# aicell-lab/bioengine-worker

Hardware: AMD Instinct MI355X
Metric: cellpose_cyto3_512x512_imgs_per_sec (higher is better)
Workload: dtype bf16; 1 GPU; model=cellpose-cyto3 CPnet (nbase 2-32-64-128-256, style on, BN folded), global_batch=32, parallelism=dp1 (replica per GPU)

## Files before the change

bioengine_worker_amd/models/cpnet.py:

```python
from __future__ import annotations

import torch
import torch.nn as nn
import torch.nn.functional as F

import os

from ..ops import conv as convops
from ..ops import conv_pair as pairops
from ..ops import style as styleops


def _norm(c: int, kind: str) -> nn.Module:
    if kind == "batch":
        return nn.BatchNorm2d(c, eps=1e-5, momentum=0.05)
    if kind == "group":
        g = 8 if c % 8 == 0 else 1
        return nn.GroupNorm(g, c, eps=1e-5)
    raise ValueError(kind)


def batchconv(cin, cout, sz, norm="batch"):
    return nn.Sequential(_norm(cin, norm), nn.ReLU(inplace=True), nn.Conv2d(cin, cout, sz, padding=sz // 2))

# ... 115 lines not shown
        T0 = self.downsample(data)
        style = self.make_style(T0[-1])
        style0 = style
        if not self.style_on:
            style = style * 0
        T1 = self.upsample(style, T0)
        T1 = self.output(T1)
        return T1, style0, T0

    def randomize_(self, seed: int = 0) -> "CPnet":
        g = torch.Generator().manual_seed(seed)
        for m in self.modules():
            if isinstance(m, nn.Conv2d):
                fan_in = m.in_channels * m.kernel_size[0] * m.kernel_size[1]
                m.weight.data = torch.randn(m.weight.shape, generator=g) * (1.0 / fan_in) ** 0.5
                if m.bias is not None:
                    m.bias.data = torch.randn(m.bias.shape, generator=g) * 0.01
            elif isinstance(m, nn.Linear):
                m.weight.data = torch.randn(m.weight.shape, generator=g) * (1.0 / m.in_features) ** 0.5
                m.bias.data = torch.randn(m.bias.shape, generator=g) * 0.01
            elif isinstance(m, nn.BatchNorm2d):
                m.weight.data = 1.0 + 0.1 * torch.randn(m.weight.shape, generator=g)
                m.bias.data = 0.1 * torch.randn(m.bias.shape, generator=g)
                m.running_mean.data = 0.1 * torch.randn(m.running_mean.shape, generator=g)
                m.running_var.data = 1.0 + 0.1 * torch.rand(m.running_var.shape, generator=g)
            elif isinstance(m, nn.GroupNorm):
                m.weight.data = 1.0 + 0.1 * torch.randn(m.weight.shape, generator=g)
                m.bias.data = 0.1 * torch.randn(m.bias.shape, generator=g)
        return self



def _bn_fold(bn: nn.Module, device) -> tuple[torch.Tensor, torch.Tensor]:
    if isinstance(bn, nn.BatchNorm2d):
        s = bn.weight.detach().float() / torch.sqrt(bn.running_var.detach().float() + bn.eps)
        t = bn.bias.detach().float() - bn.running_mean.detach().float() * s
        return s.to(device).contiguous(), t.to(device).contiguous()
    raise TypeError("CPnetEngine folds eval-mode BatchNorm only; GroupNorm nets run the autograd path")


def _pad_vec(v: torch.Tensor, n: int, fill: float) -> torch.Tensor:
    if v.numel() == n:
        return v
    out = torch.full((n,), fill, dtype=v.dtype, device=v.device)
    out[: v.numel()] = v
    return out


class _FConv:

    def __init__(self, seq: nn.Sequential, relu: bool, device, cin_pad=None, cout_pad_to=None):
        bn, conv = seq[0], seq[-1]
        self.pc = convops.PackedConv.from_weight(conv.weight, conv.bias, cin_pad=cin_pad, cout_pad_to=cout_pad_to).to(device)
        if (convops.frag_eligible(self.pc) or convops.frag_eligible_pool(self.pc) or
                convops.frag_eligible_proj(self.pc)) and torch.device(device).type == "cuda":
            self.pc.frag()
        s, t = _bn_fold(bn, device)
        self.scale = _pad_vec(s, self.pc.cin_pad, 0.0)
        self.shift = _pad_vec(t, self.pc.cin_pad, 0.0)
        self.relu = relu

    def __call__(self, x, *, x2=None, shift=None, residual=None, inmode="none", out_nchw_f32=False, cout_valid=None,
                 residual_mode="full"):
        return convops.fused_conv2d(x, self.pc, x2=x2, scale=self.scale, shift=self.shift if shift is None else shift,
                                    relu=self.relu, residual=residual, inmode=inmode, out_nchw_f32=out_nchw_f32,
                                    cout_valid=cout_valid, residual_mode=residual_mode)


class _PPConv:

    def __init__(self, conv: nn.Conv2d, device):
        from ..ops import gemm_pp as ppops

        self.cout = conv.weight.shape[0]
        self.wp = ppops.pack_conv3(conv.weight).to(device)
        self.bias = None if conv.bias is None else conv.bias.detach().float().to(device).contiguous()
        cfg = os.environ.get("BE_CPNET_PP_CFG")
        self.cfg = None if cfg is None else int(cfg)


def _igc(x, pk, **kw):
    if isinstance(pk, _PPConv):
        from ..ops import gemm_pp as ppops

        return ppops.conv3(x, pk.wp, pk.bias, cfg=pk.cfg, **kw)
    from ..ops import conv_igemm as igops

    return igops.conv3_igemm(x, pk, **kw)


class CPnetEngine:

    def __init__(self, net: CPnet, device):
        net = net.eval()
        self.device = torch.device(device)
        self.nout = net.nout
        self.nchan = net.nchan
        self.cin_pad = convops._round_up(net.nchan, 8)
        d = self.device
        self.down = []
        for n, blk in enumerate(net.downsample.down):
            cin_pad = self.cin_pad if n == 0 else None
            self.down.append(dict(
                proj=_FConv(blk.proj, False, d, cin_pad),
                c0=_FConv(blk.conv[0], True, d, cin_pad),
                c1=_FConv(blk.conv[1], True, d),
                c2=_FConv(blk.conv[2], True, d),
                c3=_FConv(blk.conv[3], True, d),
# ... 80 lines not shown
                if cfg in pairops.PROJ_CONFIGS:
                    sp.frag_proj(sp.pa.wp.device)
        return pairs

    def _build_igemm(self, net: CPnet) -> dict:
        from ..ops import conv_igemm as igops
        from ..ops import gemm_pp as ppops

        ig = {}

        def add(key, conv: nn.Conv2d):
            cout, cin, kh, _ = conv.weight.shape
            if self.ig_kind == "pp":
                if kh == 3 and ppops.conv3_supported(cin, cout):
                    ig[key] = _PPConv(conv, self.device)
            elif kh == 3 and cin % 16 == 0 and cout % 64 == 0:
                ig[key] = igops.IgemmConv.from_weight(conv.weight, conv.bias).to(self.device)

        nup = len(net.upsample.up)
        for n, blk in enumerate(net.downsample.down):
            if ("down", n, 0) in self.pair or n == 0:
                continue
            for k in (1, 2, 3):
                add(("down", n, k), blk.conv[k][-1])
        for i, blk in enumerate(net.upsample.up):
            if ("up", i, 0) in self.pair:
                continue
            if i == nup - 1:
                add(("up", i, 0), blk.conv[0][-1])
            for k in (1, 2, 3):
                add(("up", i, k), blk.conv[k].conv[-1])
        levels = {}
        for (kind, idx, k) in ig:
            levels.setdefault((kind, idx), set()).add(k)
        full = {lv for lv, ks in levels.items() if ks >= {1, 2, 3}}
        only = os.environ.get("BE_CPNET_IGEMM_LEVELS", "3")
        if only:
            keep = {int(v) for v in only.split(",") if v.strip()}
            full = {lv for lv in full if lv[1] in keep}
        return {key: v for key, v in ig.items() if (key[0], key[1]) in full}

    def _ig_level(self, kind: str, idx: int, x: torch.Tensor, H: int, W: int) -> bool:
        from ..ops import conv_igemm as igops

        pk = self.ig.get((kind, idx, 1))
        if pk is None or not x.is_cuda:
            return False
        if isinstance(pk, _PPConv):
            return True
        return igops.supported(x.shape[0], H, W, pk.cout, pk.bn)

    def _down_ig(self, n: int, e: dict, src: torch.Tensor, next_act=None) -> torch.Tensor:
        ig = self.ig
        proj = e["proj"](src, inmode="pool2")
        c1, c2, c3 = e["c1"], e["c2"], e["c3"]
        ha = convops.fused_conv2d(src, e["c0"].pc, scale=e["c0"].scale, shift=e["c0"].shift, relu=True, inmode="pool2",
                                  post_scale=c1.scale, post_shift=c1.shift, post_relu=True)
        x1, x1a = _igc(ha, ig[("down", n, 1)], residual=proj, ascale=c2.scale, ashift=c2.shift)
        _, h2a = _igc(x1a, ig[("down", n, 2)], want_out=False, ascale=c3.scale, ashift=c3.shift)
        if next_act is None:
            xd, _ = _igc(h2a, ig[("down", n, 3)], residual=x1)
            return xd, None
        return _igc(h2a, ig[("down", n, 3)], residual=x1, ascale=next_act[0], ashift=next_act[1])

    def _up_ig(self, i: int, e: dict, xcur: torch.Tensor, y: torch.Tensor, shifts: dict, xcur_act=None):
        ig = self.ig
        c1, c2, c3 = e["c1"], e["c2"], e["c3"]
        if ("up", i, 0) in ig:
            proj = e["proj"](xcur)
            _, h0a = _igc(xcur_act, ig[("up", i, 0)], residual=y, want_out=False, ascale=c1.scale,
                                       ashift=shifts[(i, 1)])
        else:
            proj = e["proj"](xcur, inmode="up2")
            h0a = convops.fused_conv2d(xcur, e["c0"].pc, scale=e["c0"].scale, shift=e["c0"].shift, relu=True,
                                       inmode="up2", residual=y, post_scale=c1.scale, post_shift=shifts[(i, 1)],
                                       post_relu=True)
        x1, x1a = _igc(h0a, ig[("up", i, 1)], residual=proj, ascale=c2.scale, ashift=shifts[(i, 2)])
        _, h2a = _igc(x1a, ig[("up", i, 2)], want_out=False, ascale=c3.scale, ashift=shifts[(i, 3)])
        out, _ = _igc(h2a, ig[("up", i, 3)], residual=x1)
        return out

    def _style_shifts(self, style: torch.Tensor) -> dict:
        st = style if self.style_on else torch.zeros_like(style)
        return self._split_shifts(styleops.style_shifts(st, self.style_w, self.style_b, self.style_s, self.style_t))

    def _split_shifts(self, shifts_all: torch.Tensor) -> dict:
        out = {}
        for (i, k, off, c) in self._feat_slices:
            out[(i, k)] = shifts_all[:, off: off + c]
        return out

    @torch.no_grad()
    def forward(self, x: torch.Tensor):
        xd = []
        h = x
        P = self.pair
        nup = len(self.up)
        top_act = None
        for n, e in enumerate(self.down):
            im = "pool2" if n > 0 else "none"
            src = x if n == 0 else xd[-1]
            if n > 0 and ("down", n, 1) in self.ig and self._ig_level("down", n, src, src.shape[1] // 2,
                                                                       src.shape[2] // 2):
                last = n == len(self.down) - 1 and ("up", nup - 1, 0) in self.ig
                nxt = (self.up[nup - 1]["c0"].scale, self.up[nup - 1]["c0"].shift) if last else None
                xdn, top_act = self._down_ig(n, e, src, nxt)
                xd.append(xdn)
                continue
            if ("down", n, 0) in P:
                if n == 0:
# ... 59 lines not shown
```

bioengine_worker_amd/ops/conv.py:

```python
from __future__ import annotations

import os

from dataclasses import dataclass

import torch
import torch.nn.functional as F

from . import _native

CK_1X1 = 64

INMODES = {"none": 0, "up2": 1, "pool2": 2}


def _round_up(v: int, m: int) -> int:
    return (v + m - 1) // m * m


@dataclass
class PackedConv:

    w: torch.Tensor
    bias: torch.Tensor | None
# ... 28 lines not shown
                    cout_pad_to: int | None = None, exact_cin: bool = False, ck16: bool = False) -> "PackedConv":
        cout, cin, ks, ks2 = weight.shape
        assert ks == ks2 and ks in (1, 3), "only 1x1 / 3x3 convs"
        cin_pad = cin_pad or _round_up(cin, 8)
        if cin_pad % 32 and cin_pad != 8 and not (exact_cin and cin_pad % 8 == 0):
            cin_pad = _round_up(cin_pad, 32)
        ck, tco = cls.choose(cin_pad, cout, ks)
        if ck16 and ks == 3 and ck == 8 and cin_pad % 16 == 0:
            ck = 16
        cout_k = max(cout, cout_pad_to or 0)
        cout_pad = _round_up(cout_k, tco)
        kp = ((ks * ks * ck + 31) // 32) * 32
        w = weight.detach().float()
        pc = cls(w=w, bias=None if bias is None else bias.detach().float(), ks=ks, cin=cin, cin_pad=cin_pad,
                 cout=cout, cout_pad=cout_pad, ck=ck, tco=tco, kp=kp)
        pc.wp = pc._pack(w)
        return pc

    def _pack(self, w: torch.Tensor) -> torch.Tensor:
        ks, ck = self.ks, self.ck
        nchunk = self.cin_pad // ck
        wz = torch.zeros(self.cout_pad, self.cin_pad, ks, ks, dtype=torch.float32, device=w.device)
        wz[: self.cout, : self.cin] = w
        t = wz.permute(0, 2, 3, 1).reshape(self.cout_pad, ks * ks, nchunk, ck)
        t = t.permute(0, 2, 1, 3).reshape(self.cout_pad, nchunk, ks * ks * ck)
        if self.kp > ks * ks * ck:
            t = F.pad(t, (0, self.kp - ks * ks * ck))
        return t.to(torch.bfloat16).contiguous()

    def to(self, device) -> "PackedConv":
        self.w = self.w.to(device)
        if self.bias is not None:
            self.bias = self.bias.to(device)
        built = self.wp is not None and self.frag_built() is not None
        if self.wp is not None:
            self.wp = self.wp.to(device)
        if built:
            self.wf = self.wf.to(device)
            self.wf_key = self._wp_key()
        return self

    def refresh(self, weight: torch.Tensor, bias: torch.Tensor | None = None) -> None:
        self.w = weight.detach().float()
        if bias is not None:
            self.bias = bias.detach().float()
        self.wp = self._pack(self.w)
        self.wf = self.wf_key = None

    def _wp_key(self) -> tuple:
        return (self.wp.data_ptr(), self.wp._version, str(self.wp.device))

    def frag(self) -> torch.Tensor:
        if self.frag_built() is None:
            self.wf = pack_frag(self.wp) if self.ks == 3 else pack_frag_1x1(self.wp)
            self.wf_key = self._wp_key()
        return self.wf

    def frag_built(self) -> torch.Tensor | None:
        if self.wf is not None and self.wf_key == self._wp_key() and self.wf.device == self.wp.device:
            return self.wf
        return None


def frag_eligible(pc: PackedConv) -> bool:
    return pc.ks == 3 and pc.ck == 32 and pc.cin_pad == 128 and pc.cout == 128 and pc.cout_pad == 128


def frag_eligible_pool(pc: PackedConv) -> bool:
    return pc.ks == 3 and pc.ck == 32 and pc.cin_pad == 64 and pc.cout == 128 and pc.cout_pad == 128


def frag_eligible_proj(pc: PackedConv) -> bool:
    return pc.ks == 1 and pc.cin_pad == 64 and pc.cout == 128 and pc.cout_pad == 128


def pp128_takes_pool(pc: PackedConv, x: torch.Tensor) -> bool:
    if not x.is_cuda or not frag_eligible_pool(pc) or pc.frag_built() is None:
        return False
    N, Hs, Ws, _ = x.shape
    return bool(_native.hip().be_conv_pp128_takes_pool(N, Hs, Ws))


def pp128_takes_pool_proj(pc: PackedConv, pp: PackedConv, x: torch.Tensor) -> bool:
    if not x.is_cuda or not frag_eligible_pool(pc) or not frag_eligible_proj(pp):
        return False
    if pc.frag_built() is None or pp.frag_built() is None:
        return False
    N, Hs, Ws, _ = x.shape
    return bool(_native.hip().be_conv_pp128_takes_pool_proj(N, Hs, Ws))


def pack_frag_1x1(wp: torch.Tensor) -> torch.Tensor:
    cout, nchunk, kp = wp.shape
    assert cout % 16 == 0 and nchunk * kp == 64, "fragment packing: a 1x1 conv of 64 input channels, whole channel tiles"
    nct = cout // 16
    t = wp.reshape(nct, 16, 2, 4, 8)
    return t.permute(2, 0, 3, 1, 4).contiguous().reshape(2, nct, 64, 8)


def pack_frag(wp: torch.Tensor) -> torch.Tensor:
    cout, nchunk, kp = wp.shape
    assert cout % 16 == 0 and kp == 288, "fragment packing: 3x3 taps of 32-channel chunks, whole channel tiles"
    nct = cout // 16
    t = wp.reshape(nct, 16, nchunk, 9, 4, 8)
    return t.permute(2, 3, 0, 4, 1, 5).contiguous().reshape(nchunk, 9, nct, 64, 8)


def unpack_frag(wf: torch.Tensor) -> torch.Tensor:
    nchunk, _, nct = wf.shape[:3]
    t = wf.reshape(nchunk, 9, nct, 4, 16, 8)
    return t.permute(2, 4, 0, 1, 3, 5).contiguous().reshape(nct * 16, nchunk, 288)


register = _native.register_hip_signatures


def _act_ref(x, x2, scale, shift, relu, inmode):
    xt = x.permute(0, 3, 1, 2)
    if inmode == "up2":
        xt = F.interpolate(xt, scale_factor=2, mode="nearest")
    elif inmode == "pool2":
        xt = F.max_pool2d(xt, 2, 2)
    if x2 is not None:
        xt = xt + x2.permute(0, 3, 1, 2).float()
    C = xt.shape[1]
    if scale is not None:
        xt = xt * (scale.view(-1, C, 1, 1) if scale.dim() == 2 else scale.view(1, C, 1, 1))
    if shift is not None:
        sh = shift.view(-1, C, 1, 1) if shift.dim() == 2 else shift.view(1, C, 1, 1)
        xt = xt + sh
    if relu:
        xt = torch.relu(xt)
    return xt


def fused_conv2d_ref(x, pc: PackedConv, x2=None, scale=None, shift=None, relu=False, residual=None,
                     inmode="none", out_nchw_f32=False, cout_valid=None, act_dtype=torch.bfloat16, post_relu=False,
                     no_bias=False):
    a = _act_ref(x.float(), x2, scale, shift, relu, inmode)
    if act_dtype is not None:
        a = a.to(act_dtype).float()
    w = pc.w.to(a.device)
    if w.shape[1] < a.shape[1]:
        w = F.pad(w, (0, 0, 0, 0, 0, a.shape[1] - w.shape[1]))
    wq = w.to(torch.bfloat16).float() if act_dtype is not None else w
    y = F.conv2d(a, wq, None, padding=pc.ks // 2)
    if pc.bias is not None and not no_bias:
        y = y + pc.bias.to(y.device).view(1, -1, 1, 1)
    if out_nchw_f32:
        cv = cout_valid or pc.cout
        y = y[:, :cv].contiguous()
        return torch.relu(y) if post_relu else y
    y = y.permute(0, 2, 3, 1)
    if residual is not None:
        y = y + residual.float()
    if post_relu:
        y = torch.relu(y)
    return y.to(x.dtype).contiguous()
# ... 86 lines not shown
        cout_store = pc.cout_pad
    else:
        assert pc.cout % 4 == 0
        if out is None:
            out = torch.empty(N, H, W, pc.cout, device=x.device, dtype=torch.bfloat16)
        else:
            assert out.shape == (N, H, W, pc.cout) and out.dtype == torch.bfloat16 and out.is_contiguous()
        cout_store = pc.cout
    if x2 is not None:
        assert x2.shape == (N, H, W, Cin) and x2.dtype == torch.bfloat16 and x2.is_contiguous()
    if residual is not None:
        assert residual.shape == ((N, H // 2, W // 2, pc.cout) if up2 else (N, H, W, pc.cout))
        assert residual.dtype == torch.bfloat16 and residual.is_contiguous()
    pscale_ns = _affine_stride(scale, N, Cin)
    pshift_ns = _affine_stride(shift, N, Cin)
    qshift_ns = _affine_stride(post_shift, N, pc.cout)
    if post_scale is not None:
        assert post_scale.dtype == torch.float32 and post_scale.is_contiguous() and post_scale.numel() == pc.cout
    wf = pc.frag_built() if frag_eligible(pc) or (inmode == "pool2" and frag_eligible_pool(pc)) else None
    args = (
        _native.ptr(x), _native.ptr(x2), _native.ptr(scale), _native.ptr(shift), pshift_ns, pscale_ns,
        int(bool(relu)) | (2 if post_relu else 0),
        _native.ptr(pc.wp), _native.ptr(None if no_bias else pc.bias), _native.ptr(residual), _native.ptr(out),
        N, H, W, Hs, Ws, Cin, cout_store, cout_valid, pc.ks, pc.ck, pc.tco, INMODES[inmode], int(out_nchw_f32),
        int(nw or choose_nw(pc, H, W, inmode, x2 is not None)), _native.ptr(post_scale), _native.ptr(post_shift),
        qshift_ns, _native.ptr(wf),
    )
    if up2:
        _native.call("be_conv2d_nhwc_frag_res", *args, 1, _native.stream(x.device))
    else:
        _native.call("be_conv2d_nhwc_frag", *args, _native.stream(x.device))
    return out


def fused_conv2d_pool_proj(x: torch.Tensor, pc: PackedConv, pp: PackedConv, *, scale, shift, relu: bool, proj_scale,
                           proj_shift) -> tuple[torch.Tensor, torch.Tensor]:
    N, Hs, Ws, Cin = x.shape
    assert x.is_cuda and x.dtype == torch.bfloat16 and x.is_contiguous() and Cin == 64 == pc.cin_pad == pp.cin_pad
    assert frag_eligible_pool(pc) and frag_eligible_proj(pp)
    wf, wpf = pc.frag_built(), pp.frag_built()
    assert wf is not None and wpf is not None, "fragment-order weights are packed when the engine is built"
    assert proj_scale.dtype == proj_shift.dtype == torch.float32 and proj_scale.numel() == proj_shift.numel() == 64
    assert proj_scale.is_contiguous() and proj_shift.is_contiguous()
    H, W = Hs // 2, Ws // 2
    out = torch.empty(N, H, W, 128, device=x.device, dtype=torch.bfloat16)
    out2 = torch.empty(N, H, W, 128, device=x.device, dtype=torch.bfloat16)
    _native.call("be_conv_pp128_pool_proj", _native.ptr(x), _native.ptr(scale), _native.ptr(shift),
                 _affine_stride(shift, N, Cin), _affine_stride(scale, N, Cin), int(bool(relu)), _native.ptr(wf),
                 _native.ptr(pc.bias), _native.ptr(out), _native.ptr(proj_scale), _native.ptr(proj_shift), _native.ptr(wpf),
                 _native.ptr(pp.bias), _native.ptr(out2), N, Hs, Ws, _native.stream(x.device))
    return out, out2


def depth_to_space2(y: torch.Tensor, c: int) -> torch.Tensor:
    N, H, W, _ = y.shape
    return y.view(N, H, W, 2, 2, c).permute(0, 1, 3, 2, 4, 5).reshape(N, 2 * H, 2 * W, c)


def fused_conv2d_concat(xa: torch.Tensor, xb: torch.Tensor, pc: PackedConv, *, post_relu: bool = False,
                        nw: int | None = None, xb_d2s: bool = False) -> torch.Tensor:
    N, H, W, Ca = xa.shape
    Cb = xb.shape[-1] // 4 if xb_d2s else xb.shape[-1]
    if xb_d2s:
        assert xb.shape[:3] == (N, H // 2, W // 2) and H % 2 == 0 and W % 2 == 0
    else:
        assert xb.shape[:3] == (N, H, W)
    assert pc.ks == 3 and pc.cin_pad == Ca + Cb
    if not xa.is_cuda:
        xbf = depth_to_space2(xb, Cb) if xb_d2s else xb
        return fused_conv2d(torch.cat([xa, xbf], -1), pc, post_relu=post_relu)
    assert xa.dtype == xb.dtype == torch.bfloat16 and xa.is_contiguous() and xb.is_contiguous()
    assert Ca % 8 == 0 and Cb % 8 == 0 and pc.cout % 4 == 0
    if pc.wp.device != xa.device:
        pc.to(xa.device)
    out = torch.empty(N, H, W, pc.cout, device=xa.device, dtype=torch.bfloat16)
    _native.call("be_conv2d_concat", _native.ptr(xa), _native.ptr(xb), _native.ptr(pc.wp), _native.ptr(pc.bias),
                 _native.ptr(out), N, H, W, Ca, Cb, pc.cout, pc.ck, pc.tco, int(bool(post_relu)),
                 int(nw or choose_nw(pc, H, W)), int(bool(xb_d2s)), _native.stream(xa.device))
    return out
```

csrc/kernels/conv_pp128.hip:

```cpp
#include <cstdlib>

#include "common.h"

namespace {
namespace pp128 {
constexpr int TH = 8, TW = 28;
constexpr int GW = 4, GT = GW * 64, NTP = 2 * GT;
constexpr int IH = TH + 2, IW = TW + 2, IPIX = IH * IW;
constexpr int IN_B = IPIX * 64;
constexpr int LDS = 2 * IN_B;
constexpr int NF = 14, FC = 7;
constexpr int NCH = 4;
constexpr int C = 128;
constexpr int HU = IPIX * 4, HUPT = (HU + GT - 1) / GT;
constexpr int WD = 3;
constexpr int WSTEP = 8 * 64 * 8;
constexpr int BD = 6, BR = 7;
static_assert(IW % 4 == 2, "the swizzle derivation needs 30 y = 2 y (mod 4)");
constexpr int PJ_B = TH * TW * 128;
constexpr int LDS_PROJ = LDS + 2 * PJ_B;
static_assert(LDS_PROJ <= 128 * 1024, "LDS budget of the ping-pong kernels");
static_assert(BD < BR, "ring");

struct Args {
  const bf16_t* x;
  const float* sa;
  const float* ta;
  const bf16_t* wf;
  const float* bias;
  const bf16_t* res;
  bf16_t* out;
  int N, H, W;
  int sa_ns, ta_ns;
  int relu;
  int res_up2;
  int tiles_x, tiles_y;
  const float* sp;
  const float* tp;
  const bf16_t* wpf;
  const float* bias_p;
  bf16_t* out2;
  unsigned long long* stamps;
};

struct TileXY {
  int n, ty0, tx0;
};

__device__ __forceinline__ TileXY tile_of(const Args& a, int t) {
  const int tpi = a.tiles_x * a.tiles_y;
  TileXY r;
  r.n = t / tpi;
  const int q = t - r.n * tpi;
  r.ty0 = (q / a.tiles_x) * TH;
  r.tx0 = (q % a.tiles_x) * TW;
  return r;
}

template <bool POOL>
struct Halo {
  u32x4 h[HUPT];
  float4 aff[4];
};

template <>
struct Halo<true> {
  u32x4 h[HUPT], hb[HUPT];
  u32x4 q[HUPT], qb[HUPT];
  float4 aff[4];
  float4 affp[4];
};

template <bool POOL>
__device__ __forceinline__ void issue_aff(const Args& a, TileXY t, int c, Halo<POOL>& hr) {
  hr.aff[0] = hr.aff[1] = make_float4(1.f, 1.f, 1.f, 1.f);
  hr.aff[2] = hr.aff[3] = make_float4(0.f, 0.f, 0.f, 0.f);
  if (a.sa) {
    const float* sr = a.sa + (size_t)t.n * a.sa_ns + c;
    hr.aff[0] = *reinterpret_cast<const float4*>(sr);
    hr.aff[1] = *reinterpret_cast<const float4*>(sr + 4);
  }
  if (a.ta) {
    const float* tr = a.ta + (size_t)t.n * a.ta_ns + c;
    hr.aff[2] = *reinterpret_cast<const float4*>(tr);
    hr.aff[3] = *reinterpret_cast<const float4*>(tr + 4);
  }
}

__device__ __forceinline__ size_t pool_src(const Args& a, int n, int gy, int gx, int row, int c) {
  return (((size_t)n * 2 * a.H + 2 * gy + row) * 2 * a.W + 2 * gx) * 64 + c;
}

template <bool POOL>
__device__ __forceinline__ void issue_halo(const Args& a, TileXY t, int ch, int gt, Halo<POOL>& hr) {
  const int c = ch * 32 + (gt & 3) * 8;
// ... 198 lines not shown
  const __amdgpu_buffer_rsrc_t rb = __builtin_amdgcn_make_buffer_rsrc(
      const_cast<float*>(a.bias ? a.bias : a.sa), (short)0, a.bias ? C * 4 : 0, 0x00020000);
  auto voff = [&](int j, int y, int x) {
    if constexpr (FULL) return (((t.ty0 + y) * a.W + t.tx0 + x) * C + co) * 2;
    const int py = t.ty0 + 4 * (j / FC) + y, px = t.tx0 + 4 * (j % FC) + x;
    return (py < a.H && px < a.W) ? ((py * a.W + px) * C + co) * 2 : 0x7ffffff0;
  };
  auto soff = [&](int j) { return FULL ? ((j / FC) * 4 * a.W + (j % FC) * 4) * C * 2 : 0; };
  auto voff_r = [&](int j, int y, int x) {
    if constexpr (FULL) return ((((t.ty0 + y) >> 1) * Wr + ((t.tx0 + x) >> 1)) * C + co) * 2;
    const int py = t.ty0 + 4 * (j / FC) + y, px = t.tx0 + 4 * (j % FC) + x;
    return (py < a.H && px < a.W) ? (((py >> 1) * Wr + (px >> 1)) * C + co) * 2 : 0x7ffffff0;
  };
  auto soff_r = [&](int j) { return FULL ? ((j / FC) * 2 * Wr + (j % FC) * 2) * C * 2 : 0; };
  u32x2 rv[RES ? NF : 1][2];
  f32x4 bias[2];
#pragma unroll
  for (int ct = 0; ct < 2; ++ct)
    bias[ct] = __builtin_bit_cast(f32x4, __builtin_amdgcn_raw_buffer_load_b128(rb, (co + ct * 16) * 4, 0, 0));
  if constexpr (RES != 0) {
#pragma unroll
    for (int j = 0; j < NF; ++j) {
      const int o = RES == 2 ? voff_r(j, ly, lx) : voff(j, ly, lx);
      const int so = RES == 2 ? soff_r(j) : soff(j);
#pragma unroll
      for (int ct = 0; ct < 2; ++ct) rv[j][ct] = __builtin_amdgcn_raw_buffer_load_b64(rr, o + ct * 32, so, 0);
    }
  } else {
#pragma unroll
    for (int ct = 0; ct < 2; ++ct) bias[ct] = bias[ct] + (f32x4){0.f, 0.f, 0.f, 0.f};
  }
  __builtin_amdgcn_sched_barrier(0);
  int sy = ly, sx = lx;
  asm volatile("" : "+v"(sy), "+v"(sx));
#pragma unroll
  for (int j = 0; j < NF; ++j) {
    const int o = act ? voff(j, sy, sx) : 0x7ffffff0;
#pragma unroll
    for (int ct = 0; ct < 2; ++ct) {
      u32x2 st;
      if constexpr (RES != 0) {
        const u32x2 r = rv[j][ct];
        st[0] = pack2bf(acc[ct][j][0] + bias[ct][0] + lo_bf(r[0]), acc[ct][j][1] + bias[ct][1] + hi_bf(r[0]));
        st[1] = pack2bf(acc[ct][j][2] + bias[ct][2] + lo_bf(r[1]), acc[ct][j][3] + bias[ct][3] + hi_bf(r[1]));
      } else {
        st[0] = pack2bf(acc[ct][j][0] + bias[ct][0], acc[ct][j][1] + bias[ct][1]);
        st[1] = pack2bf(acc[ct][j][2] + bias[ct][2], acc[ct][j][3] + bias[ct][3]);
      }
      __builtin_amdgcn_raw_buffer_store_b64(st, ro, o + ct * 32, soff(j), 0);
    }
  }
}

template <bool STAMP = false, bool POOL = false, bool PROJ = false>
__global__ __launch_bounds__(NTP, 2) void conv_pp128_kernel(Args a) {
  static_assert(POOL || !PROJ, "the projection reads the pooled input");
  constexpr int NC = POOL ? 2 : NCH;
  unsigned long long ph_work[5] = {0, 0, 0, 0, 0}, ph_wait[5] = {0, 0, 0, 0, 0};
  unsigned long long tstamp = STAMP ? __builtin_amdgcn_s_memtime() : 0;
  auto pre = [&](int i) {
    if constexpr (STAMP) {
      const unsigned long long tn = __builtin_amdgcn_s_memtime();
      ph_work[i] += tn - tstamp;
      tstamp = tn;
    }
  };
  auto post = [&](int i) {
    if constexpr (STAMP) {
      const unsigned long long tn = __builtin_amdgcn_s_memtime();
      ph_wait[i] += tn - tstamp;
      tstamp = tn;
    }
  };
  auto slot = [](int c) { return c > 0 ? 2 : 0; };
  extern __shared__ __attribute__((aligned(16))) unsigned char smem[];
  const int tid0 = threadIdx.x;
  const int total = a.N * a.tiles_x * a.tiles_y;
  const int t0 = (int)(((long long)blockIdx.x * total) / gridDim.x);
  const int t1 = (int)(((long long)(blockIdx.x + 1) * total) / gridDim.x);
  if (t0 >= t1) return;
  const int grp = __builtin_amdgcn_readfirstlane(tid0 / GT);
  const int gt0 = tid0 & (GT - 1);
  unsigned char* reg = smem + grp * IN_B;
  unsigned char* rpj = PROJ ? smem + LDS + grp * PJ_B : nullptr;
  Halo<POOL> halo;
  issue_halo(a, tile_of(a, min(t0 + grp, t1 - 1)), 0, gt0, halo);
  if constexpr (POOL) issue_halo_b(a, tile_of(a, min(t0 + grp, t1 - 1)), 0, gt0, halo);
  if constexpr (PROJ) issue_affp(a, 0, gt0, halo);
  if (grp == 1) __builtin_amdgcn_s_barrier();
  const int iters = (t1 - t0 + 1) >> 1;
  for (int k = 0; k < iters; ++k) {
    int gt = gt0;
    asm volatile("" : "+v"(gt));
    const int cp = __builtin_amdgcn_readfirstlane(gt >> 6), lane = gt & 63, lrow = lane & 15, kq = lane >> 4;
    const int t = t0 + 2 * k + grp;
    const bool act = t < t1;
    const TileXY cur = tile_of(a, act ? t : t1 - 1);
    const bf16_t* wl = w_lane(a.wf, cp, lane);
    int A0[3];
#pragma unroll
    for (int dx = 0; dx < 3; ++dx) {
      const int x = (lrow & 3) + dx;
      A0[dx] = ((lrow >> 2) * IW + x) * 64 + ((kq ^ (((x >> 1) & 1) << 1)) << 4);
    }
    f32x4 acc[2][NF];
#pragma unroll
    for (int i = 0; i < 2; ++i)
#pragma unroll
      for (int j = 0; j < NF; ++j) acc[i][j] = (f32x4){0.f, 0.f, 0.f, 0.f};
    WPre wpre;
#pragma unroll
    for (int c = 0; c < NC; ++c) {
      int gc = gt0;
      asm volatile("" : "+v"(gc));
      if constexpr (POOL) {
        reduce_a(halo);
        if (c > 0) {
          __builtin_amdgcn_sched_barrier(0);
          issue_halo_b(a, cur, c, gc, halo);
        }
        reduce_b(halo);
        if constexpr (PROJ) {
          if (c > 0) {
            __builtin_amdgcn_sched_barrier(0);
            issue_affp(a, c, gc, halo);
          }
        }
      }
      commit(a, cur, gc, halo, reg);
      if constexpr (PROJ) {
        __builtin_amdgcn_sched_barrier(0);
        commit_proj(c, gc, halo, rpj);
      }
      __builtin_amdgcn_sched_barrier(0);
      if (c + 1 < NC)
        issue_halo(a, cur, c + 1, gc, halo);
      else
        issue_halo(a, tile_of(a, min(t + 2, t1 - 1)), 0, gc, halo);
      issue_w(wl + c * 9 * WSTEP, wpre);
      pre(slot(c));
      __syncthreads();
      post(slot(c));
      __builtin_amdgcn_s_setprio(1);
      mma_chunk(acc, reg, wl + c * 9 * WSTEP, wpre, A0);
      __builtin_amdgcn_s_setprio(0);
      pre(slot(c) + 1);
      __syncthreads();
      post(slot(c) + 1);
    }
    int g3 = gt0;
    asm volatile("" : "+v"(g3));
    const bool full = cur.ty0 + TH <= a.H && cur.tx0 + TW <= a.W;
    if constexpr (POOL) {
      if constexpr (!PROJ) {
        issue_halo_b(a, tile_of(a, min(t + 2, t1 - 1)), 0, g3, halo);
        __builtin_amdgcn_sched_barrier(0);
      }
      if (full)
        epilogue<0, true>(a, cur, acc, cp, g3 & 15, (g3 & 63) >> 4, act);
      else
        epilogue<0, false>(a, cur, acc, cp, g3 & 15, (g3 & 63) >> 4, act);
      if constexpr (PROJ) {
        __builtin_amdgcn_sched_barrier(0);
        int g4 = gt0;
        asm volatile("" : "+v"(g4));
        proj_mma(acc, rpj, w_lane(a.wpf, cp, g4 & 63), g4 & 15, (g4 & 63) >> 4);
        Args b = a;
        b.out = a.out2;
        b.bias = a.bias_p;
        if (full)
          epilogue<0, true>(b, cur, acc, cp, g4 & 15, (g4 & 63) >> 4, act);
        else
          epilogue<0, false>(b, cur, acc, cp, g4 & 15, (g4 & 63) >> 4, act);
        __builtin_amdgcn_sched_barrier(0);
        issue_halo_b(a, tile_of(a, min(t + 2, t1 - 1)), 0, g4, halo);
        issue_affp(a, 0, g4, halo);
      }
    } else if (a.res != nullptr && a.res_up2) {
      if (full)
        epilogue<2, true>(a, cur, acc, cp, g3 & 15, (g3 & 63) >> 4, act);
      else
        epilogue<2, false>(a, cur, acc, cp, g3 & 15, (g3 & 63) >> 4, act);
    } else if (a.res != nullptr) {
      if (full)
        epilogue<1, true>(a, cur, acc, cp, g3 & 15, (g3 & 63) >> 4, act);
      else
        epilogue<1, false>(a, cur, acc, cp, g3 & 15, (g3 & 63) >> 4, act);
    } else {
      if (full)
        epilogue<0, true>(a, cur, acc, cp, g3 & 15, (g3 & 63) >> 4, act);
      else
        epilogue<0, false>(a, cur, acc, cp, g3 & 15, (g3 & 63) >> 4, act);
    }
    pre(4);
    __syncthreads();
    post(4);
  }
  if (grp == 0) __builtin_amdgcn_s_barrier();
  if constexpr (STAMP) {
    if ((tid0 & (GT - 1)) < 16) {
      const int k = tid0 & 15;
      unsigned long long v = 0;
#pragma unroll
      for (int i = 0; i < 5; ++i) {
        if (k == i) v = ph_work[i];
        if (k == 8 + i) v = ph_wait[i];
      }
      if (k == 15) v = (unsigned long long)iters;
      a.stamps[((size_t)blockIdx.x * 2 + grp) * 16 + k] = v;
    }
  }
}
}

int g_pp128 = [] {
  const char* e = getenv("BE_CONV_PP128");
  return e ? atoi(e) : 1;
}();

int g_pp128_res_up2 = [] {
  const char* e = getenv("BE_CONV_PP128_RES_UP2");
  return e ? atoi(e) : 1;
}();

int g_pp128_pool = [] {
  const char* e = getenv("BE_CONV_PP128_POOL");
  return e ? atoi(e) : 1;
}();

int g_pp128_pool_proj = [] {
  const char* e = getenv("BE_CONV_PP128_POOL_PROJ");
  return e ? atoi(e) : 1;
}();

int g_pp128_grid = 0;
int g_pp128_launches = 0;
int g_pp128_pool_launches = 0;
unsigned long long* g_pp128_stamps = nullptr;
int g_pp128_stamps_cap = 0;

int pp128_grid_for(int N, int H, int W, int* tiles_x, int* tiles_y) {
  if (!g_pp128 || N <= 0 || H <= 0 || W <= 0 || (long long)H * W * 256 >= (1LL << 31) - 64) return 0;
  const int tx = (W + pp128::TW - 1) / pp128::TW, ty = (H + pp128::TH - 1) / pp128::TH;
  const long long tiles = (long long)N * tx * ty;
  const bool forced = g_pp128_grid > 0;
  const int g = forced ? (int)(tiles < g_pp128_grid ? tiles : g_pp128_grid) : 256;
  if (!(forced || tiles >= 2LL * g) || tiles >= (1LL << 30)) return 0;
  if (tiles_x) *tiles_x = tx;
  if (tiles_y) *tiles_y = ty;
  return g;
}

}

extern "C" {

int be_conv2d_nhwc(const void* x, const void* x2, const float* pscale, const float* pshift, int pshift_ns, int pscale_ns,
                   int prelu, const void* w, const float* bias, const void* res, void* out, int N, int H, int W,
                   int Hs, int Ws, int Cin, int Cout, int cout_valid, int ks, int ck, int tco, int inmode,
                   int out_f32_nchw, int nw, const float* qscale, const float* qshift, int qshift_ns,
                   hipStream_t stream);

int be_conv_pp128_set_grid(int blocks) {
  g_pp128_grid = blocks;
  return 0;
}

int be_conv_pp128_set_stamps(void* buf, int cap_workgroups) {
  g_pp128_stamps = static_cast<unsigned long long*>(buf);
  g_pp128_stamps_cap = buf ? cap_workgroups : 0;
  return 0;
}

int be_conv_pp128_launches() { return g_pp128_launches; }

int be_conv2d_nhwc_frag_res(const void* x, const void* x2, const float* pscale, const float* pshift, int pshift_ns,
                            int pscale_ns, int prelu, const void* w, const float* bias, const void* res, void* out,
                            int N, int H, int W, int Hs, int Ws, int Cin, int Cout, int cout_valid, int ks, int ck,
                            int tco, int inmode, int out_f32_nchw, int nw, const float* qscale, const float* qshift,
                            int qshift_ns, const void* wfrag, int res_up2, hipStream_t stream) {
  const bool shape_ok = wfrag && ks == 3 && ck == 32 && inmode == 0 && !x2 && !out_f32_nchw && Cin == 128 &&
                        Cout == 128 && Hs == H && Ws == W && !(prelu & 2) && !qscale && !qshift && x && out;
  if (res_up2 && !(shape_ok && res && H % 2 == 0 && W % 2 == 0)) return -31;
  const bool pool_ok = g_pp128_pool && wfrag && ks == 3 && ck == 32 && inmode == 2 && !x2 && !out_f32_nchw && Cin == 64 &&
                       Cout == 128 && Hs == 2 * H && Ws == 2 * W && !(prelu & 2) && !qscale && !qshift && !res && x && out;
  if (shape_ok || pool_ok) {
    pp128::Args a;
    const int g = pp128_grid_for(N, H, W, &a.tiles_x, &a.tiles_y);
    if (g > 0 && pool_ok) {
      a.x = (const bf16_t*)x; a.sa = pscale; a.ta = pshift; a.sa_ns = pscale_ns; a.ta_ns = pshift_ns;
      a.wf = (const bf16_t*)wfrag; a.bias = bias; a.res = nullptr; a.out = (bf16_t*)out;
      a.N = N; a.H = H; a.W = W; a.relu = prelu & 1;
      a.res_up2 = 0;
      a.sp = a.tp = a.bias_p = nullptr; a.wpf = nullptr; a.out2 = nullptr;
      a.stamps = g_pp128_stamps;
      ++g_pp128_pool_launches;
      if (g_pp128_stamps != nullptr) {
// ... 37 lines not shown
}

int be_conv_pp128_takes(int N, int H, int W) { return pp128_grid_for(N, H, W, nullptr, nullptr) > 0 ? 1 : 0; }

int be_conv_pp128_takes_pool(int N, int Hs, int Ws) {
  return g_pp128_pool && Hs % 2 == 0 && Ws % 2 == 0 && pp128_grid_for(N, Hs / 2, Ws / 2, nullptr, nullptr) > 0 ? 1 : 0;
}

int be_conv_pp128_set_pool(int pool, int pool_proj) {
  g_pp128_pool = pool;
  g_pp128_pool_proj = pool_proj;
  return 0;
}

int be_conv_pp128_pool_launches() { return g_pp128_pool_launches; }

int be_conv_pp128_takes_pool_proj(int N, int Hs, int Ws) {
  return g_pp128_pool_proj && be_conv_pp128_takes_pool(N, Hs, Ws);
}

int be_conv_pp128_pool_proj(const void* x, const float* pscale, const float* pshift, int pshift_ns, int pscale_ns, int prelu,
                            const void* wfrag, const float* bias, void* out, const float* sp, const float* tp,
                            const void* wpfrag, const float* bias_p, void* out2, int N, int Hs, int Ws,
                            hipStream_t stream) {
  if (!x || !wfrag || !out || !sp || !tp || !wpfrag || !out2 || out == out2 || (prelu & ~1)) return -32;
  if (!be_conv_pp128_takes_pool_proj(N, Hs, Ws)) return -32;
  pp128::Args a;
  const int g = pp128_grid_for(N, Hs / 2, Ws / 2, &a.tiles_x, &a.tiles_y);
  a.x = (const bf16_t*)x; a.sa = pscale; a.ta = pshift; a.sa_ns = pscale_ns; a.ta_ns = pshift_ns;
  a.wf = (const bf16_t*)wfrag; a.bias = bias; a.res = nullptr; a.out = (bf16_t*)out;
  a.N = N; a.H = Hs / 2; a.W = Ws / 2; a.relu = prelu & 1;
  a.res_up2 = 0;
  a.sp = sp; a.tp = tp; a.wpf = (const bf16_t*)wpfrag; a.bias_p = bias_p; a.out2 = (bf16_t*)out2;
  a.stamps = g_pp128_stamps;
  static bool attr_set[BE_MAX_DEV] = {};
  if (!attr_set[be_cur_dev()]) {
    if (hipFuncSetAttribute(reinterpret_cast<const void*>(&pp128::conv_pp128_kernel<false, true, true>),
                            hipFuncAttributeMaxDynamicSharedMemorySize, pp128::LDS_PROJ) != hipSuccess ||
        hipFuncSetAttribute(reinterpret_cast<const void*>(&pp128::conv_pp128_kernel<true, true, true>),
                            hipFuncAttributeMaxDynamicSharedMemorySize, pp128::LDS_PROJ) != hipSuccess)
      return -33;
    attr_set[be_cur_dev()] = true;
  }
  ++g_pp128_pool_launches;
  if (g_pp128_stamps != nullptr) {
    if (g > g_pp128_stamps_cap) return -30;
    hipLaunchKernelGGL((pp128::conv_pp128_kernel<true, true, true>), dim3(g), dim3(pp128::NTP), pp128::LDS_PROJ, stream, a);
    return BE_CHECK_LAUNCH();
  }
  hipLaunchKernelGGL((pp128::conv_pp128_kernel<false, true, true>), dim3(g), dim3(pp128::NTP), pp128::LDS_PROJ, stream, a);
  return BE_CHECK_LAUNCH();
}

int be_conv_pp128_takes_res_up2(int N, int H, int W) {
  return g_pp128_res_up2 && H % 2 == 0 && W % 2 == 0 && be_conv_pp128_takes(N, H, W);
}

}
```

Baseline: 2488 img/s.

## Pre-pool level-3 input and run c0 conv through 256-channel pp128 kernel

New measurement: 2544 img/s (median of 6 runs). 1.02x the previous value.

```diff
diff --git a/bioengine_worker_amd/models/cpnet.py b/bioengine_worker_amd/models/cpnet.py
--- a/bioengine_worker_amd/models/cpnet.py
+++ b/bioengine_worker_amd/models/cpnet.py
@@ -191,8 +191,8 @@
     def __init__(self, seq: nn.Sequential, relu: bool, device, cin_pad=None, cout_pad_to=None):
         bn, conv = seq[0], seq[-1]
         self.pc = convops.PackedConv.from_weight(conv.weight, conv.bias, cin_pad=cin_pad, cout_pad_to=cout_pad_to).to(device)
-        if (convops.frag_eligible(self.pc) or convops.frag_eligible_pool(self.pc) or
-                convops.frag_eligible_proj(self.pc)) and torch.device(device).type == "cuda":
+        if (convops.frag_eligible(self.pc) or convops.frag_eligible_pool(self.pc) or convops.frag_eligible_proj(self.pc)
+                or convops.frag_eligible_c256(self.pc)) and torch.device(device).type == "cuda":
             self.pc.frag()
         s, t = _bn_fold(bn, device)
         self.scale = _pad_vec(s, self.pc.cin_pad, 0.0)
@@ -379,10 +379,21 @@
 
     def _down_ig(self, n: int, e: dict, src: torch.Tensor, next_act=None) -> torch.Tensor:
         ig = self.ig
-        proj = e["proj"](src, inmode="pool2")
-        c1, c2, c3 = e["c1"], e["c2"], e["c3"]
-        ha = convops.fused_conv2d(src, e["c0"].pc, scale=e["c0"].scale, shift=e["c0"].shift, relu=True, inmode="pool2",
-                                  post_scale=c1.scale, post_shift=c1.shift, post_relu=True)
+        c0, c1, c2, c3 = e["c0"], e["c1"], e["c2"], e["c3"]
+        entry = convops.pp128_pooled_entry(c0.pc, src)
+        if entry:
+            pooled = convops.pool2_nhwc(src)
+            proj = e["proj"](pooled)
+            if entry == 2:
+                ha = convops.fused_conv2d_c256(pooled, c0.pc, scale=c0.scale, shift=c0.shift, relu=True,
+                                               post_scale=c1.scale, post_shift=c1.shift, post_relu=True)
+            else:
+                ha = convops.fused_conv2d(pooled, c0.pc, scale=c0.scale, shift=c0.shift, relu=True, nw=8,
+                                          post_scale=c1.scale, post_shift=c1.shift, post_relu=True)
+        else:
+            proj = e["proj"](src, inmode="pool2")
+            ha = convops.fused_conv2d(src, c0.pc, scale=c0.scale, shift=c0.shift, relu=True, inmode="pool2",
+                                      post_scale=c1.scale, post_shift=c1.shift, post_relu=True)
         x1, x1a = _igc(ha, ig[("down", n, 1)], residual=proj, ascale=c2.scale, ashift=c2.shift)
         _, h2a = _igc(x1a, ig[("down", n, 2)], want_out=False, ascale=c3.scale, ashift=c3.shift)
         if next_act is None:
diff --git a/bioengine_worker_amd/ops/conv.py b/bioengine_worker_amd/ops/conv.py
--- a/bioengine_worker_amd/ops/conv.py
+++ b/bioengine_worker_amd/ops/conv.py
@@ -104,7 +104,10 @@
 
     def frag(self) -> torch.Tensor:
         if self.frag_built() is None:
-            self.wf = pack_frag(self.wp) if self.ks == 3 else pack_frag_1x1(self.wp)
+            if frag_eligible_c256(self):
+                self.wf = pack_frag_c256(self.wp)
+            else:
+                self.wf = pack_frag(self.wp) if self.ks == 3 else pack_frag_1x1(self.wp)
             self.wf_key = self._wp_key()
         return self.wf
 
@@ -124,6 +127,33 @@
 
 def frag_eligible_proj(pc: PackedConv) -> bool:
     return pc.ks == 1 and pc.cin_pad == 64 and pc.cout == 128 and pc.cout_pad == 128
+
+
+def frag_eligible_c256(pc: PackedConv) -> bool:
+    return pc.ks == 3 and pc.ck == 32 and pc.cin_pad == 128 and pc.cout == 256 and pc.cout_pad == 256
+
+
+def pp128_takes_prepool(pc: PackedConv, x: torch.Tensor) -> bool:
+    if not x.is_cuda or not frag_eligible_c256(pc):
+        return False
+    N, Hs, Ws, _ = x.shape
+    if Hs % 2 or Ws % 2:
+        return False
+    return bool(_native.hip().be_conv_pp128_takes_prepool(N, Hs // 2, Ws // 2))
+
+
+def pp128_takes_c256(pc: PackedConv, x: torch.Tensor) -> bool:
+    if not x.is_cuda or not frag_eligible_c256(pc) or pc.frag_built() is None:
+        return False
+    N, H, W, _ = x.shape
+    return bool(_native.hip().be_conv_pp128_takes_c256(N, H, W))
+
+
+def pp128_pooled_entry(pc: PackedConv, x: torch.Tensor) -> int:
+    if not pp128_takes_prepool(pc, x):
+        return 0
+    N, Hs, Ws, _ = x.shape
+    return 2 if pc.frag_built() is not None and _native.hip().be_conv_pp128_takes_c256(N, Hs // 2, Ws // 2) else 1
 
 
 def pp128_takes_pool(pc: PackedConv, x: torch.Tensor) -> bool:
@@ -156,6 +186,12 @@
     nct = cout // 16
     t = wp.reshape(nct, 16, nchunk, 9, 4, 8)
     return t.permute(2, 3, 0, 4, 1, 5).contiguous().reshape(nchunk, 9, nct, 64, 8)
+
+
+def pack_frag_c256(wp: torch.Tensor) -> torch.Tensor:
+    cout, nchunk, kp = wp.shape
+    assert cout == 256 and nchunk == 4 and kp == 288, "fragment packing: a 3x3 conv of 128 -> 256 channels"
+    return torch.stack([pack_frag(wp[:128]), pack_frag(wp[128:])]).contiguous()
 
 
 def unpack_frag(wf: torch.Tensor) -> torch.Tensor:
@@ -348,6 +384,48 @@
     return out, out2
 
 
+def pool2_nhwc_ref(x: torch.Tensor) -> torch.Tensor:
+    def mx(p, q):
+        return torch.where((p > q) | ((p == q) & ~torch.signbit(p)), p, q)
+
+    return mx(mx(x[:, 0::2, 0::2], x[:, 0::2, 1::2]), mx(x[:, 1::2, 0::2], x[:, 1::2, 1::2])).contiguous()
+
+
+def pool2_nhwc(x: torch.Tensor, out: torch.Tensor | None = None) -> torch.Tensor:
+    N, Hs, Ws, C = x.shape
+    assert Hs % 2 == 0 and Ws % 2 == 0, "pool2_nhwc needs an even source size"
+    if not x.is_cuda:
+        y = pool2_nhwc_ref(x)
+        if out is not None:
+            out.copy_(y)
+            return out
+        return y
+    assert x.dtype == torch.bfloat16 and x.is_contiguous() and C % 8 == 0, "pool2_nhwc expects contiguous NHWC bf16"
+    if out is None:
+        out = torch.empty(N, Hs // 2, Ws // 2, C, device=x.device, dtype=torch.bfloat16)
+    else:
+        assert out.shape == (N, Hs // 2, Ws // 2, C) and out.dtype == torch.bfloat16 and out.is_contiguous()
+    _native.call("be_pool2_nhwc", _native.ptr(x), _native.ptr(out), N, Hs, Ws, C, _native.stream(x.device))
+    return out
+
+
+def fused_conv2d_c256(x: torch.Tensor, pc: PackedConv, *, scale, shift, relu: bool, post_scale, post_shift,
+                      post_relu: bool) -> torch.Tensor:
+    N, H, W, Cin = x.shape
+    assert x.is_cuda and x.dtype == torch.bfloat16 and x.is_contiguous() and Cin == 128 == pc.cin_pad
+    assert frag_eligible_c256(pc)
+    wf = pc.frag_built()
+    assert wf is not None, "fragment-order weights are packed when the engine is built"
+    for q in (post_scale, post_shift):
+        assert q is not None and q.dtype == torch.float32 and q.is_contiguous() and q.dim() == 1 and q.numel() == 256
+    out = torch.empty(N, H, W, 256, device=x.device, dtype=torch.bfloat16)
+    _native.call("be_conv_pp128_c256", _native.ptr(x), _native.ptr(scale), _native.ptr(shift),
+                 _affine_stride(shift, N, Cin), _affine_stride(scale, N, Cin), int(bool(relu)) | (2 if post_relu else 0),
+                 _native.ptr(wf), _native.ptr(pc.bias), _native.ptr(out), _native.ptr(post_scale), _native.ptr(post_shift),
+                 N, H, W, _native.stream(x.device))
+    return out
+
+
 def depth_to_space2(y: torch.Tensor, c: int) -> torch.Tensor:
     N, H, W, _ = y.shape
     return y.view(N, H, W, 2, 2, c).permute(0, 1, 3, 2, 4, 5).reshape(N, 2 * H, 2 * W, c)
diff --git a/csrc/kernels/conv_pp128.hip b/csrc/kernels/conv_pp128.hip
--- a/csrc/kernels/conv_pp128.hip
+++ b/csrc/kernels/conv_pp128.hip
@@ -41,6 +41,9 @@
   const float* bias_p;
   bf16_t* out2;
   unsigned long long* stamps;
+  const float* qs = nullptr;
+  const float* qt = nullptr;
+  int qrelu = 0;
 };
 
 struct TileXY {
@@ -345,9 +348,58 @@
   }
 }
 
-template <bool STAMP = false, bool POOL = false, bool PROJ = false>
+template <bool FULL>
+__device__ __forceinline__ void epilogue_c256(const Args& a, TileXY t, int half, const f32x4 (&acc)[2][NF], int cp, int lrow,
+                                              int kq, bool act) {
+  constexpr int CO = 2 * C;
+  const int ly = lrow >> 2, lx = lrow & 3;
+  const int co = half * C + cp * 32 + kq * 4;
+  const int img_b = a.H * a.W * CO * 2;
+  const __amdgpu_buffer_rsrc_t ro =
+      __builtin_amdgcn_make_buffer_rsrc(a.out + (size_t)t.n * a.H * a.W * CO, (short)0, img_b, 0x00020000);
+  const __amdgpu_buffer_rsrc_t rb = __builtin_amdgcn_make_buffer_rsrc(
+      const_cast<float*>(a.bias ? a.bias : a.qs), (short)0, a.bias ? CO * 4 : 0, 0x00020000);
+  const __amdgpu_buffer_rsrc_t rs = __builtin_amdgcn_make_buffer_rsrc(const_cast<float*>(a.qs), (short)0, CO * 4, 0x00020000);
+  const __amdgpu_buffer_rsrc_t rt = __builtin_amdgcn_make_buffer_rsrc(const_cast<float*>(a.qt), (short)0, CO * 4, 0x00020000);
+  auto voff = [&](int j, int y, int x) {
+    if constexpr (FULL) return (((t.ty0 + y) * a.W + t.tx0 + x) * CO + co) * 2;
+    const int py = t.ty0 + 4 * (j / FC) + y, px = t.tx0 + 4 * (j % FC) + x;
+    return (py < a.H && px < a.W) ? ((py * a.W + px) * CO + co) * 2 : 0x7ffffff0;
+  };
+  auto soff = [&](int j) { return FULL ? ((j / FC) * 4 * a.W + (j % FC) * 4) * CO * 2 : 0; };
+  f32x4 bias[2], qs[2], qt[2];
+#pragma unroll
+  for (int ct = 0; ct < 2; ++ct) {
+    bias[ct] = __builtin_bit_cast(f32x4, __builtin_amdgcn_raw_buffer_load_b128(rb, (co + ct * 16) * 4, 0, 0));
+    qs[ct] = __builtin_bit_cast(f32x4, __builtin_amdgcn_raw_buffer_load_b128(rs, (co + ct * 16) * 4, 0, 0));
+    qt[ct] = __builtin_bit_cast(f32x4, __builtin_amdgcn_raw_buffer_load_b128(rt, (co + ct * 16) * 4, 0, 0));
+    bias[ct] = bias[ct] + (f32x4){0.f, 0.f, 0.f, 0.f};
+  }
+  const bool qrelu = a.qrelu != 0;
+  __builtin_amdgcn_sched_barrier(0);
+#pragma unroll
+  for (int j = 0; j < NF; ++j) {
+    const int o = act ? voff(j, ly, lx) : 0x7ffffff0;
+#pragma unroll
+    for (int ct = 0; ct < 2; ++ct) {
+      const uint32_t p0 = pack2bf(acc[ct][j][0] + bias[ct][0], acc[ct][j][1] + bias[ct][1]);
+      const uint32_t p1 = pack2bf(acc[ct][j][2] + bias[ct][2], acc[ct][j][3] + bias[ct][3]);
+      u32x2 st;
+      st[0] = pack2bf(fmaf(lo_bf(p0), qs[ct][0], qt[ct][0]), fmaf(hi_bf(p0), qs[ct][1], qt[ct][1]));
+      st[1] = pack2bf(fmaf(lo_bf(p1), qs[ct][2], qt[ct][2]), fmaf(hi_bf(p1), qs[ct][3], qt[ct][3]));
+      if (qrelu) {
+        st[0] = relu_bf16x2(st[0]);
+        st[1] = relu_bf16x2(st[1]);
+      }
+      __builtin_amdgcn_raw_buffer_store_b64(st, ro, o + ct * 32, soff(j), 0);
+    }
+  }
+}
+
+template <bool STAMP = false, bool POOL = false, bool PROJ = false, bool C256 = false>
 __global__ __launch_bounds__(NTP, 2) void conv_pp128_kernel(Args a) {
   static_assert(POOL || !PROJ, "the projection reads the pooled input");
+  static_assert(!(POOL && C256), "the 256-channel build reads a plain 128-channel input");
   constexpr int NC = POOL ? 2 : NCH;
   unsigned long long ph_work[5] = {0, 0, 0, 0, 0}, ph_wait[5] = {0, 0, 0, 0, 0};
   unsigned long long tstamp = STAMP ? __builtin_amdgcn_s_memtime() : 0;
@@ -368,7 +420,8 @@
   auto slot = [](int c) { return c > 0 ? 2 : 0; };
   extern __shared__ __attribute__((aligned(16))) unsigned char smem[];
   const int tid0 = threadIdx.x;
-  const int total = a.N * a.tiles_x * a.tiles_y;
+  const int total = a.N * a.tiles_x * a.tiles_y * (C256 ? 2 : 1);
+  auto tile_at = [&](int item) { return tile_of(a, C256 ? item >> 1 : item); };
   const int t0 = (int)(((long long)blockIdx.x * total) / gridDim.x);
   const int t1 = (int)(((long long)(blockIdx.x + 1) * total) / gridDim.x);
   if (t0 >= t1) return;
@@ -377,8 +430,8 @@
   unsigned char* reg = smem + grp * IN_B;
   unsigned char* rpj = PROJ ? smem + LDS + grp * PJ_B : nullptr;
   Halo<POOL> halo;
-  issue_halo(a, tile_of(a, min(t0 + grp, t1 - 1)), 0, gt0, halo);
-  if constexpr (POOL) issue_halo_b(a, tile_of(a, min(t0 + grp, t1 - 1)), 0, gt0, halo);
+  issue_halo(a, tile_at(min(t0 + grp, t1 - 1)), 0, gt0, halo);
+  if constexpr (POOL) issue_halo_b(a, tile_at(min(t0 + grp, t1 - 1)), 0, gt0, halo);
   if constexpr (PROJ) issue_affp(a, 0, gt0, halo);
   if (grp == 1) __builtin_amdgcn_s_barrier();
   const int iters = (t1 - t0 + 1) >> 1;
@@ -388,8 +441,8 @@
     const int cp = __builtin_amdgcn_readfirstlane(gt >> 6), lane = gt & 63, lrow = lane & 15, kq = lane >> 4;
     const int t = t0 + 2 * k + grp;
     const bool act = t < t1;
-    const TileXY cur = tile_of(a, act ? t : t1 - 1);
-    const bf16_t* wl = w_lane(a.wf, cp, lane);
+    const TileXY cur = tile_at(act ? t : t1 - 1);
+    const bf16_t* wl = w_lane(C256 ? a.wf + ((act ? t : t1 - 1) & 1) * (NCH * 9 * WSTEP) : a.wf, cp, lane);
     int A0[3];
 #pragma unroll
     for (int dx = 0; dx < 3; ++dx) {
@@ -429,7 +482,7 @@
       if (c + 1 < NC)
         issue_halo(a, cur, c + 1, gc, halo);
       else
-        issue_halo(a, tile_of(a, min(t + 2, t1 - 1)), 0, gc, halo);
+        issue_halo(a, tile_at(min(t + 2, t1 - 1)), 0, gc, halo);
       issue_w(wl + c * 9 * WSTEP, wpre);
       pre(slot(c));
       __syncthreads();
@@ -446,7 +499,7 @@
     const bool full = cur.ty0 + TH <= a.H && cur.tx0 + TW <= a.W;
     if constexpr (POOL) {
       if constexpr (!PROJ) {
-        issue_halo_b(a, tile_of(a, min(t + 2, t1 - 1)), 0, g3, halo);
+        issue_halo_b(a, tile_at(min(t + 2, t1 - 1)), 0, g3, halo);
         __builtin_amdgcn_sched_barrier(0);
       }
       if (full)
@@ -466,9 +519,15 @@
         else
           epilogue<0, false>(b, cur, acc, cp, g4 & 15, (g4 & 63) >> 4, act);
         __builtin_amdgcn_sched_barrier(0);
-        issue_halo_b(a, tile_of(a, min(t + 2, t1 - 1)), 0, g4, halo);
+        issue_halo_b(a, tile_at(min(t + 2, t1 - 1)), 0, g4, halo);
         issue_affp(a, 0, g4, halo);
       }
+    } else if constexpr (C256) {
+      const int half = (act ? t : t1 - 1) & 1;
+      if (full)
+        epilogue_c256<true>(a, cur, half, acc, cp, g3 & 15, (g3 & 63) >> 4, act);
+      else
+        epilogue_c256<false>(a, cur, half, acc, cp, g3 & 15, (g3 & 63) >> 4, act);
     } else if (a.res != nullptr && a.res_up2) {
       if (full)
         epilogue<2, true>(a, cur, acc, cp, g3 & 15, (g3 & 63) >> 4, act);
@@ -526,16 +585,27 @@
   return e ? atoi(e) : 1;
 }();
 
+int g_l3_prepool = [] {
+  const char* e = getenv("BE_CPNET_L3_PREPOOL");
+  return e ? atoi(e) : 1;
+}();
+
+int g_pp128_c256 = [] {
+  const char* e = getenv("BE_CONV_PP128_C256");
+  return e ? atoi(e) : 1;
+}();
+
+int g_pp128_c256_launches = 0;
 int g_pp128_grid = 0;
 int g_pp128_launches = 0;
 int g_pp128_pool_launches = 0;
 unsigned long long* g_pp128_stamps = nullptr;
 int g_pp128_stamps_cap = 0;
 
-int pp128_grid_for(int N, int H, int W, int* tiles_x, int* tiles_y) {
-  if (!g_pp128 || N <= 0 || H <= 0 || W <= 0 || (long long)H * W * 256 >= (1LL << 31) - 64) return 0;
+int pp128_grid_for(int N, int H, int W, int* tiles_x, int* tiles_y, int halves = 1) {
+  if (!g_pp128 || N <= 0 || H <= 0 || W <= 0 || (long long)H * W * 256 * halves >= (1LL << 31) - 64) return 0;
   const int tx = (W + pp128::TW - 1) / pp128::TW, ty = (H + pp128::TH - 1) / pp128::TH;
-  const long long tiles = (long long)N * tx * ty;
+  const long long tiles = (long long)N * tx * ty * halves;
   const bool forced = g_pp128_grid > 0;
   const int g = forced ? (int)(tiles < g_pp128_grid ? tiles : g_pp128_grid) : 256;
   if (!(forced || tiles >= 2LL * g) || tiles >= (1LL << 30)) return 0;
@@ -679,6 +749,48 @@
   return BE_CHECK_LAUNCH();
 }
 
+static int pp128_c256_grid_for(int N, int H, int W, int* tiles_x, int* tiles_y) {
+  return pp128_grid_for(N, H, W, tiles_x, tiles_y, 2);
+}
+
+int be_conv_pp128_takes_prepool(int N, int H, int W) {
+  return g_l3_prepool && pp128_c256_grid_for(N, H, W, nullptr, nullptr) > 0 ? 1 : 0;
+}
+
+int be_conv_pp128_takes_c256(int N, int H, int W) { return g_pp128_c256 && be_conv_pp128_takes_prepool(N, H, W); }
+
+int be_conv_pp128_set_c256(int prepool, int c256) {
+  g_l3_prepool = prepool;
+  g_pp128_c256 = c256;
+  return 0;
+}
+
+int be_conv_pp128_c256_launches() { return g_pp128_c256_launches; }
+
+int be_conv_pp128_c256(const void* x, const float* pscale, const float* pshift, int pshift_ns, int pscale_ns, int prelu,
+                       const void* wfrag, const float* bias, void* out, const float* qscale, const float* qshift, int N,
+                       int H, int W, hipStream_t stream) {
+  if (!x || !wfrag || !out || x == out || !qscale || !qshift || (prelu & ~3)) return -34;
+  if (!be_conv_pp128_takes_c256(N, H, W)) return -34;
+  pp128::Args a;
+  const int g = pp128_c256_grid_for(N, H, W, &a.tiles_x, &a.tiles_y);
+  a.x = (const bf16_t*)x; a.sa = pscale; a.ta = pshift; a.sa_ns = pscale_ns; a.ta_ns = pshift_ns;
+  a.wf = (const bf16_t*)wfrag; a.bias = bias; a.res = nullptr; a.out = (bf16_t*)out;
+  a.N = N; a.H = H; a.W = W; a.relu = prelu & 1;
+  a.res_up2 = 0;
+  a.sp = a.tp = a.bias_p = nullptr; a.wpf = nullptr; a.out2 = nullptr;
+  a.qs = qscale; a.qt = qshift; a.qrelu = (prelu >> 1) & 1;
+  a.stamps = g_pp128_stamps;
+  ++g_pp128_c256_launches;
+  if (g_pp128_stamps != nullptr) {
+    if (g > g_pp128_stamps_cap) return -30;
+    hipLaunchKernelGGL((pp128::conv_pp128_kernel<true, false, false, true>), dim3(g), dim3(pp128::NTP), pp128::LDS, stream, a);
+    return BE_CHECK_LAUNCH();
+  }
+  hipLaunchKernelGGL((pp128::conv_pp128_kernel<false, false, false, true>), dim3(g), dim3(pp128::NTP), pp128::LDS, stream, a);
+  return BE_CHECK_LAUNCH();
+}
+
 int be_conv_pp128_takes_res_up2(int N, int H, int W) {
   return g_pp128_res_up2 && H % 2 == 0 && W % 2 == 0 && be_conv_pp128_takes(N, H, W);
 }
diff --git a/csrc/kernels/pool2_nhwc.hip b/csrc/kernels/pool2_nhwc.hip
--- /dev/null
+++ b/csrc/kernels/pool2_nhwc.hip
@@ -0,0 +1,42 @@
+#include "common.h"
+
+namespace {
+
+__device__ __forceinline__ uint32_t pool_max4(uint32_t r0, uint32_t r1, uint32_t q0, uint32_t q1) {
+  const float lo = fmaxf(fmaxf(lo_bf(r0), lo_bf(r1)), fmaxf(lo_bf(q0), lo_bf(q1)));
+  const float hi = fmaxf(fmaxf(hi_bf(r0), hi_bf(r1)), fmaxf(hi_bf(q0), hi_bf(q1)));
+  return (__float_as_uint(lo) >> 16) | (__float_as_uint(hi) & 0xffff0000u);
+}
+
+__global__ __launch_bounds__(256) void pool2_nhwc_kernel(const bf16_t* __restrict__ x, bf16_t* __restrict__ out,
+                                                         long long units, int H, int W, int CU) {
+  const long long u = (long long)blockIdx.x * 256 + threadIdx.x;
+  if (u >= units) return;
+  const int c = (int)(u % CU);
+  const long long p = u / CU;
+  const int px = (int)(p % W);
+  const long long ny = p / W;
+  const size_t row = (size_t)2 * W * CU;
+  const u32x4* s = reinterpret_cast<const u32x4*>(x) + (size_t)2 * ny * row + (size_t)2 * px * CU + c;
+  const u32x4 r0 = s[0], r1 = s[CU], q0 = s[row], q1 = s[row + CU];
+  u32x4 o;
+#pragma unroll
+  for (int j = 0; j < 4; ++j) o[j] = pool_max4(r0[j], r1[j], q0[j], q1[j]);
+  reinterpret_cast<u32x4*>(out)[u] = o;
+}
+
+}
+
+extern "C" {
+
+int be_pool2_nhwc(const void* x, void* out, int N, int Hs, int Ws, int C, hipStream_t stream) {
+  if (!x || !out || x == out || N <= 0 || Hs <= 0 || Ws <= 0 || C <= 0 || (Hs & 1) || (Ws & 1) || (C & 7)) return -40;
+  const long long units = (long long)N * (Hs / 2) * (Ws / 2) * (C / 8);
+  const long long blocks = (units + 255) / 256;
+  if (blocks >= (1LL << 31)) return -41;
+  hipLaunchKernelGGL(pool2_nhwc_kernel, dim3((unsigned)blocks), dim3(256), 0, stream, (const bf16_t*)x, (bf16_t*)out, units,
+                     Hs / 2, Ws / 2, C / 8);
+  return BE_CHECK_LAUNCH();
+}
+
+}
```
